# anaykulkarni/collective-communication-mpi

Measured on AMD Instinct MI355X. Metric: all-reduce algbw (GB/s) @1GiB fp32 + DP4xTP2 fwd step time, 1/2/4/8 MI355X, higher is better.
Workload: dtype fp32; 1 GPU; global_batch=2048, seq_len=16, parallelism=dp1xtp1, allreduce_algo=twoshot, allreduce_bytes=1073741824

## Files before the change

### collective_communication_mpi_amd/csrc/device/attn_common.hpp

```cpp
#pragma once
#include <cstdint>

#include <hip/hip_runtime.h>

namespace ccmpi {
namespace dev {
namespace attn {

struct AttnArgs {
  const uint16_t* qkv;
  uint16_t* o;
  float* lse;
  const uint16_t* dout;
  uint16_t* dqkv;
  float* dbias;
  int B, S, Hl, D, ld_qkv, ld_o;
  float scale;
  uint16_t* pool;
  int ld_pool;
  int dout_bstride;
  int dout_rstride;
  const uint16_t* wo;
  int ld_wo, n_out;
  float* zp;
  int ld_zp;
  const float* bo;
  const uint16_t* dz;
  int ld_dz;
  float dz_scale;
  float* ztok;
  int ld_zt;
  int zrows;
  float* zpush[16];
  const uint16_t* xq;
  int ld_xq, kq;
  const uint16_t* wq;
  int ld_wq;
  const float* bq;
  uint16_t* qkv_out;
  const float* img;
  uint16_t* xq_out;
  const float* fold_wq;
  int ld_fold_wq;
  const float* fold_we;
  int ld_fold_we;
  uint16_t* fold_out;
  int ld_fold_out, fold_R, fold_d, fold_kp;
  int fold_at_start;
  int fold_sched;
  unsigned long long* tstamp;
};
constexpr int kTStamps = 32;

bool mfma_supported(const AttnArgs& a, bool bwd);
void launch_fwd_mfma(const AttnArgs& a, hipStream_t stream);
void launch_bwd_mfma(const AttnArgs& a, hipStream_t stream);
void launch_qkv_fwd_mfma(const AttnArgs& a, hipStream_t stream);
extern int g_qkv_grid_cap;
extern int g_qkv_fold_sched;
extern int g_qkv_fold_grid;
extern int g_bwd_grid_cap;

}
}
}
```

### collective_communication_mpi_amd/csrc/device/attn_mfma.hip

```cpp
#include <hip/hip_runtime.h>

#include <algorithm>
#include <cstdlib>

#include "attn_common.hpp"
#include "common.hpp"

namespace ccmpi {
namespace dev {
void fold_emb_qkv_mfma(const float* Wq, int ld_wq, const float* We, int ld_we, uint16_t* Weff, int ld_eff, int R, int d,
                       int kp, hipStream_t stream);
namespace attn {
namespace {

typedef __bf16 bf16x8 __attribute__((ext_vector_type(8)));
typedef short s4 __attribute__((ext_vector_type(4)));
typedef float f4 __attribute__((ext_vector_type(4)));
constexpr int WPB = 4;

__device__ __forceinline__ s4 pack4(float a, float b, float c, float d) {
  const uint2 u{pk_bf16(a, b), pk_bf16(c, d)};
  return __builtin_bit_cast(s4, u);
}
__device__ __forceinline__ bf16x8 ld_row16(const uint16_t* p, bool ok) {
// ... 799 lines not shown
    }
    store_tile<D, LD>(Ot, acc, a.scale, gq, a.ld_qkv, S, lane);
  }
  if (a.dbias) {
    float* red = reinterpret_cast<float*>(sm);
    __syncthreads();
#pragma unroll
    for (int nt = 0; nt < NT; ++nt) {
      float q = bq[nt], k = bk[nt], v = bv[nt];
      q = pair32_sum(pair16_sum(q));
      k = pair32_sum(pair16_sum(k));
      v = pair32_sum(pair16_sum(v));
      if (g == 0) {
        red[(wave * 3 + 0) * D + 16 * nt + c] = q;
        red[(wave * 3 + 1) * D + 16 * nt + c] = k;
        red[(wave * 3 + 2) * D + 16 * nt + c] = v;
      }
    }
    __syncthreads();
    for (int i = threadIdx.x; i < 3 * D; i += blockDim.x) {
      float acc = 0.f;
#pragma unroll
      for (int w = 0; w < WPB; ++w) acc += red[w * 3 * D + i];
      atomicAdd(a.dbias + (i / D) * HD + h * D + i % D, acc);
    }
  }
}

template <int D>
constexpr size_t bwd_lds_bytes() {
  return (size_t)WPB * 4 * 16 * (D + 8) * sizeof(uint16_t);
}

int grid_for(int npairs, int cap, int nw = WPB) { return std::max(1, std::min((npairs + nw - 1) / nw, cap)); }

}

bool mfma_supported(const AttnArgs& a, bool bwd) {
  if (a.S < 1 || a.S > 16 || !(a.D == 32 || a.D == 64 || a.D == 128)) return false;
  if (a.ld_qkv % 8 || a.ld_o % 8 || ((uint64_t)a.qkv % 16) || ((uint64_t)a.o % 16)) return false;
  if (bwd && (a.dout_bstride % 8 || a.dout_rstride % 8 || ((uint64_t)a.dout % 16) || ((uint64_t)a.dqkv % 16))) return false;
  return true;
}

void launch_fwd_mfma(const AttnArgs& a, hipStream_t stream) {
  const int grid = grid_for(a.B * a.Hl, 4096);
  if (a.D == 32) hipLaunchKernelGGL(k_attn16_fwd<32>, dim3(grid), dim3(256), 0, stream, a);
  else if (a.D == 64) hipLaunchKernelGGL(k_attn16_fwd<64>, dim3(grid), dim3(256), 0, stream, a);
  else hipLaunchKernelGGL(k_attn16_fwd<128>, dim3(grid), dim3(256), 0, stream, a);
}

int g_qkv_grid_cap = std::getenv("CCMPI_QKV_GRID") ? std::atoi(std::getenv("CCMPI_QKV_GRID")) : 256;

constexpr double kFoldRounds = 1.5;
int g_qkv_fold_sched = -1;
int g_qkv_fold_grid = 1;

bool fold_sched_on() {
  if (g_qkv_fold_sched < 0) {
    const char* e = std::getenv("CCMPI_QKV_FOLD_SCHED");
    g_qkv_fold_sched = (e && std::atoi(e) == 0) ? 0 : 1;
  }
  return g_qkv_fold_sched != 0;
}

int fold_sched_for(const AttnArgs& a, int grid) {
// ... 36 lines not shown
  const dim3 block(64 * kQkvWaves);
  AttnArgs a = args;
  const bool fold_apart = a.fold_out && fold_tiles_n > grid;
  if (fold_apart) a.fold_out = nullptr;
  a.fold_sched = fold_sched_for(a, grid);
  const bool train = a.lse || a.qkv_out || a.xq_out || a.pool;
  const bool lean = a.ld_wq == 72 && (!a.fold_out || a.fold_at_start);
  if (a.tstamp) launch_qkv_variant<true, true, false>(a, grid, block, stream);
  else if (lean) (train ? launch_qkv_variant<false, true, true> : launch_qkv_variant<false, false, true>)(a, grid, block, stream);
  else (train ? launch_qkv_variant<false, true, false> : launch_qkv_variant<false, false, false>)(a, grid, block, stream);
  if (fold_apart)
    fold_emb_qkv_mfma(args.fold_wq, args.ld_fold_wq, args.fold_we, args.ld_fold_we, args.fold_out, args.ld_fold_out,
                      args.fold_R, args.fold_d, args.fold_kp, stream);
}

int g_bwd_grid_cap = 0;

void launch_bwd_mfma(const AttnArgs& a, hipStream_t stream) {
  int grid = grid_for(a.B * a.Hl, a.dbias ? (g_bwd_grid_cap > 0 ? g_bwd_grid_cap : 256 * a.Hl) : 4096);
  grid = std::max(a.Hl, grid / a.Hl * a.Hl);
  if (a.D == 32) {
    hipLaunchKernelGGL(k_attn16_bwd<32>, dim3(grid), dim3(256), bwd_lds_bytes<32>(), stream, a);
  } else if (a.D == 64) {
    hipLaunchKernelGGL(k_attn16_bwd<64>, dim3(grid), dim3(256), bwd_lds_bytes<64>(), stream, a);
  } else {
    static bool attr = hipFuncSetAttribute(reinterpret_cast<const void*>(k_attn16_bwd<128>),
                                           hipFuncAttributeMaxDynamicSharedMemorySize,
                                           (int)bwd_lds_bytes<128>()) == hipSuccess;
    (void)attr;
    hipLaunchKernelGGL(k_attn16_bwd<128>, dim3(grid), dim3(256), bwd_lds_bytes<128>(), stream, a);
  }
}

}
}
}
```

### collective_communication_mpi_amd/csrc/device/attn_small.hip

```cpp
#include <pybind11/pybind11.h>
#include <pybind11/stl.h>

#include <tuple>
#include <vector>

#include "attn_common.hpp"
#include "common.hpp"
#include "ops.hpp"

namespace ccmpi {
namespace dev {

namespace {
using attn::AttnArgs;

__device__ __forceinline__ float ld_bf16(const uint16_t* p) { return __uint_as_float((uint32_t)(*p) << 16); }
__device__ __forceinline__ void st_bf16(uint16_t* p, float v) { *p = (uint16_t)f32_to_bf16_bits(v); }

__device__ __forceinline__ float wave_max(float v) {
  for (int o = 32; o > 0; o >>= 1) v = fmaxf(v, __shfl_xor(v, o));
  return v;
}
__device__ __forceinline__ float wave_sum(float v) {
  for (int o = 32; o > 0; o >>= 1) v += __shfl_xor(v, o);
// ... 162 lines not shown
        atomicAdd(&colsum[2 * D + d], dv);
      }
    }
  }
  if (a.dbias && fixed_col && threadIdx.x < S * D) {
    const int d = threadIdx.x % D;
    atomicAdd(&colsum[d], sq);
    atomicAdd(&colsum[D + d], sk);
    atomicAdd(&colsum[2 * D + d], sv);
  }
  if (a.dbias) {
    __syncthreads();
    for (int c = threadIdx.x; c < 3 * D; c += blockDim.x) {
      const int part = c / D, d = c % D;
      atomicAdd(a.dbias + part * HD + h * D + d, colsum[c]);
    }
  }
}

size_t fwd_lds(int S, int D) { return sizeof(float) * (3 * S * (D + 1) + S * (S + 1)); }
size_t bwd_lds(int S, int D) { return sizeof(float) * (5 * S * (D + 1) + 2 * S * (S + 1) + S + 3 * D); }

void check_dims(int S, int D, bool bwd) {
  if (S < 1 || S > 64 || D < 1 || D > 256) throw std::invalid_argument("attn_small: need 1 <= S <= 64, D <= 256");
  if ((bwd ? bwd_lds(S, D) : fwd_lds(S, D)) > 160 * 1024) throw std::invalid_argument("attn_small: tile exceeds LDS");
}

static void check_fused_fc(const AttnArgs& a, bool bwd) {
  if (!attn::mfma_supported(a, bwd) || a.n_out < 1 || a.n_out > 16 || 4 % a.Hl || !a.wo)
    throw std::invalid_argument("attention: fused fc_o needs S <= 16, D in {32, 64, 128}, Hl | 4, n_out <= 16");
  if (bwd && (a.ld_dz < 16 || a.ld_dz % 8 || ((uint64_t)a.dz % 16)))
    throw std::invalid_argument("attention: fused fc_o backward needs dz rows of >= 16 bf16, 16-B aligned");
  if (!bwd && !a.pool) throw std::invalid_argument("attention: fused fc_o forward needs the pooled output");
}

void attn_fwd(uint64_t qkv, uint64_t o, uint64_t lse, int B, int S, int Hl, int D, int ld_qkv, int ld_o, float scale,
              uint64_t pool, int ld_pool, uint64_t stream, uint64_t wo, int ld_wo, int n_out, uint64_t zp, int ld_zp,
              uint64_t bo, uint64_t ztok, int ld_zt, int zrows, const std::vector<uint64_t>& zpush) {
  check_dims(S, D, false);
  AttnArgs a{(const uint16_t*)qkv, (uint16_t*)o, (float*)lse, nullptr, nullptr, nullptr, B, S, Hl, D, ld_qkv, ld_o, scale,
             (uint16_t*)pool, ld_pool, 0, 0, (const uint16_t*)wo, ld_wo, n_out, (float*)zp, ld_zp, (const float*)bo,
             nullptr, 0, 1.0f};
  if (zp) check_fused_fc(a, false);
  if (ztok || zrows) {
    if (zp || !attn::mfma_supported(a, false) || n_out < 1 || n_out > 16 || 4 % Hl || !wo || ld_wo % 8 ||
        (wo % 16) || ld_zt < 16 || ld_zt % 4 || (ztok % 16))
      throw std::invalid_argument("attention: per-token fused fc_o needs S <= 16, D in {32, 64, 128}, Hl | 4, "
                                  "n_out <= 16, 16-B aligned W_o rows, z rows of >= 16 floats");
    if (zrows) {
      const int64_t M = (int64_t)B * S;
      const int64_t blocks = M / zrows;
      if (zrows % S || M % zrows || blocks < 1 || blocks > 16 || (int64_t)zpush.size() != blocks)
        throw std::invalid_argument("attention: push fc_o needs whole sequences per block (zrows % S == 0), "
                                    "B*S = blocks x zrows and one target per block (<= 16)");
      for (int64_t j = 0; j < blocks; ++j) {
        if (!zpush[j] || zpush[j] % 16) throw std::invalid_argument("attention: push fc_o targets must be 16-B aligned");
        a.zpush[j] = reinterpret_cast<float*>(zpush[j]);
      }
    }
    a.ztok = reinterpret_cast<float*>(ztok);
    a.ld_zt = ld_zt;
    a.zrows = zrows;
  }
  if (attn::mfma_supported(a, false)) {
    attn::launch_fwd_mfma(a, (hipStream_t)stream);
    CCMPI_HIP_CHECK(hipGetLastError());
// ... 30 lines not shown
  a.lse = (float*)lse;
  a.tstamp = (unsigned long long*)tstamp;
  a.B = B; a.S = S; a.Hl = Hl; a.D = D; a.ld_qkv = ld_qkv; a.scale = scale;
  a.pool = (uint16_t*)pool; a.ld_pool = ld_pool;
  a.wo = (const uint16_t*)wo; a.ld_wo = ld_wo; a.n_out = n_out; a.bo = (const float*)bo;
  a.xq = (const uint16_t*)xq; a.ld_xq = ld_xq; a.kq = kq;
  a.wq = (const uint16_t*)wq; a.ld_wq = ld_wq; a.bq = (const float*)bq; a.qkv_out = (uint16_t*)qkv_out;
  a.img = (const float*)img; a.xq_out = (uint16_t*)xq_out;
  a.zp = (float*)zmean; a.ld_zp = ld_zmean;
  a.fold_wq = (const float*)fold_wq; a.ld_fold_wq = ld_fold_wq; a.fold_we = (const float*)fold_we;
  a.ld_fold_we = ld_fold_we; a.fold_out = (uint16_t*)fold_out; a.ld_fold_out = ld_fold_out;
  a.fold_R = fold_R; a.fold_d = fold_d; a.fold_kp = kq;
  static const int at_start = std::getenv("CCMPI_FOLD_TAIL_AT") && std::string(std::getenv("CCMPI_FOLD_TAIL_AT")) == "end" ? 0 : 1;
  a.fold_at_start = at_start;
  a.ztok = (float*)ztok; a.ld_zt = ld_zt; a.zrows = zrows;
  if (zrows) {
    const int64_t M = (int64_t)B * S;
    const int64_t blocks = M / zrows;
    if (zrows % S || M % zrows || blocks < 1 || blocks > 16 || (int64_t)zpush.size() != blocks)
      throw std::invalid_argument("attention: push fc_o needs whole sequences per block (zrows % S == 0), "
                                  "B*S = blocks x zrows and one target per block (<= 16)");
    for (int64_t j = 0; j < blocks; ++j) {
      if (!zpush[j] || zpush[j] % 16) throw std::invalid_argument("attention: push fc_o targets must be 16-B aligned");
      a.zpush[j] = reinterpret_cast<float*>(zpush[j]);
    }
  }
  if (B == 0) return;
  attn::launch_qkv_fwd_mfma(a, (hipStream_t)stream);
  CCMPI_HIP_CHECK(hipGetLastError());
}

void attn_bwd(uint64_t qkv, uint64_t o, uint64_t lse, uint64_t dout, uint64_t dqkv, uint64_t dbias, int B, int S,
              int Hl, int D, int ld_qkv, int ld_o, float scale, int dout_bstride, int dout_rstride, uint64_t stream,
              uint64_t dz, int ld_dz, uint64_t wo, int ld_wo, int n_out, float dz_scale) {
  check_dims(S, D, true);
  AttnArgs a{(const uint16_t*)qkv, (uint16_t*)o, (float*)lse, (const uint16_t*)dout, (uint16_t*)dqkv, (float*)dbias,
             B, S, Hl, D, ld_qkv, ld_o, scale, nullptr, 0, dout_bstride, dout_rstride, (const uint16_t*)wo, ld_wo,
             n_out, nullptr, 0, nullptr, (const uint16_t*)dz, ld_dz, dz_scale};
  if (dz) check_fused_fc(a, true);
  if (attn::mfma_supported(a, true)) {
    attn::launch_bwd_mfma(a, (hipStream_t)stream);
    CCMPI_HIP_CHECK(hipGetLastError());
    return;
  }
  hipLaunchKernelGGL(k_attn_bwd, dim3(B * Hl), dim3(256), bwd_lds(S, D), (hipStream_t)stream, a);
  CCMPI_HIP_CHECK(hipGetLastError());
}

constexpr int kMaxT = 4, kTT = 32;
struct TRegions {
  uint64_t off[kMaxT], rows[kMaxT], cols[kMaxT];
  uint16_t* dst[kMaxT];
  int tiles[kMaxT + 1];
  int n;
};

__device__ __forceinline__ bool in_regions(const TRegions& tr, uint64_t i) {
  for (int k = 0; k < tr.n; ++k)
    if (i >= tr.off[k] && i - tr.off[k] < tr.rows[k] * tr.cols[k]) return true;
  return false;
}

struct AdamArgs {
  float* p;
  float* g;
  float* m;
  float* v;
  uint16_t* p16;
  uint64_t n;
  float lr, b1, b2, eps, wd, bc1, bc2, grad_scale;
  int zero_grad;
  int* step_dev;
// ... 207 lines not shown
void register_attn_ops(pybind11::module_& m) {
  m.def("rows_mean", &rows_mean, "out[g] = mean of fp32 rows z[g S .. g S + S) (ordered sum)", pybind11::arg("z"),
        pybind11::arg("ld_z"), pybind11::arg("out"), pybind11::arg("ld_out"), pybind11::arg("groups"),
        pybind11::arg("S"), pybind11::arg("ncol"), pybind11::arg("stream"),
        pybind11::call_guard<pybind11::gil_scoped_release>());
  m.def("attn_set_qkv_grid", [](int cap) { attn::g_qkv_grid_cap = cap > 0 ? cap : 256; },
        "workgroups of the fused QKV forward (default 256: one 8-wave workgroup per CU)", pybind11::arg("cap"));
  m.def("attn_set_qkv_fold_sched", [](int v) { attn::g_qkv_fold_sched = v < 0 ? -1 : (v ? 1 : 0); },
        "fused QKV forward with the in-kernel fold: 1 = fold owners take fewer pair blocks, 0 = grid-stride, "
        "-1 = CCMPI_QKV_FOLD_SCHED (default 1)", pybind11::arg("v"));
  m.def("attn_set_qkv_fold_grid", [](int v) { attn::g_qkv_fold_grid = v ? 1 : 0; },
        "fused QKV forward with the in-kernel fold: 1 = at small batches the grid grows by the fold's tiles "
        "(fold-only workgroups beside the attention ones), 0 = not (ranks sharing one GPU)", pybind11::arg("v"));
  m.def("attn_set_bwd_grid", [](int cap) { attn::g_bwd_grid_cap = cap > 0 ? cap : 0; },
        "backward kernel grid cap (tuning)");
  namespace py = pybind11;
  m.def("attn_small_fwd", &attn_fwd, py::arg("qkv"), py::arg("o"), py::arg("lse"), py::arg("B"), py::arg("S"),
        py::arg("Hl"), py::arg("D"), py::arg("ld_qkv"), py::arg("ld_o"), py::arg("scale"), py::arg("pool"),
        py::arg("ld_pool"), py::arg("stream"), py::arg("wo") = 0, py::arg("ld_wo") = 0, py::arg("n_out") = 0,
        py::arg("zp") = 0, py::arg("ld_zp") = 0, py::arg("bo") = 0, py::arg("ztok") = 0, py::arg("ld_zt") = 16,
        py::arg("zrows") = 0, py::arg("zpush") = std::vector<uint64_t>{}, py::call_guard<py::gil_scoped_release>());
  m.def("attn_qkv_fwd", &attn_qkv_fwd, py::arg("xq"), py::arg("ld_xq"), py::arg("kq"), py::arg("wq"), py::arg("ld_wq"),
        py::arg("bq"), py::arg("qkv_out"), py::arg("ld_qkv"), py::arg("lse"), py::arg("B"), py::arg("S"), py::arg("Hl"),
        py::arg("D"), py::arg("scale"), py::arg("pool"), py::arg("ld_pool"), py::arg("wo"), py::arg("ld_wo"),
        py::arg("n_out"), py::arg("bo"), py::arg("ztok"), py::arg("ld_zt"), py::arg("zrows"), py::arg("zpush"),
        py::arg("stream"), py::arg("img") = 0, py::arg("xq_out") = 0, py::arg("zmean") = 0, py::arg("ld_zmean") = 16,
        py::arg("fold_wq") = 0, py::arg("ld_fold_wq") = 0, py::arg("fold_we") = 0, py::arg("ld_fold_we") = 0,
        py::arg("fold_out") = 0, py::arg("ld_fold_out") = 0, py::arg("fold_R") = 0, py::arg("fold_d") = 0,
        py::arg("tstamp") = 0, py::call_guard<py::gil_scoped_release>());
  m.def("attn_small_bwd", &attn_bwd, py::arg("qkv"), py::arg("o"), py::arg("lse"), py::arg("dout"), py::arg("dqkv"),
        py::arg("dbias"), py::arg("B"), py::arg("S"), py::arg("Hl"), py::arg("D"), py::arg("ld_qkv"), py::arg("ld_o"),
        py::arg("scale"), py::arg("dout_bstride"), py::arg("dout_rstride"), py::arg("stream"), py::arg("dz") = 0,
        py::arg("ld_dz") = 0, py::arg("wo") = 0, py::arg("ld_wo") = 0, py::arg("n_out") = 0,
        py::arg("dz_scale") = 1.0f, py::call_guard<py::gil_scoped_release>());
  m.def("adamw_step", &adamw, py::arg("p"), py::arg("g"), py::arg("m"), py::arg("v"), py::arg("p16"), py::arg("n"),
        py::arg("lr"), py::arg("b1"), py::arg("b2"), py::arg("eps"), py::arg("wd"), py::arg("step"),
        py::arg("grad_scale"), py::arg("stream"),
        py::arg("tregions") = std::vector<std::tuple<uint64_t, uint64_t, uint64_t, uint64_t>>{},
        py::arg("zero_grad") = false, py::arg("step_dev") = 0, py::arg("step_parity") = 0, py::call_guard<py::gil_scoped_release>());
  m.def("cast_bf16", &cast_bf16, py::arg("x"), py::arg("y"), py::arg("n"), py::arg("stream"),
        py::arg("tregions") = std::vector<std::tuple<uint64_t, uint64_t, uint64_t, uint64_t>>{},
        py::call_guard<py::gil_scoped_release>());
  m.def("patchify", &patchify, py::arg("x"), py::arg("xp"), py::arg("B"), py::arg("img"), py::arg("p"), py::arg("kp"),
        py::arg("stream"), py::arg("ldo") = 0, py::call_guard<py::gil_scoped_release>());
}

}
}
```

### collective_communication_mpi_amd/models/mnist_tp.py

```python
from __future__ import annotations

import math
import os
from dataclasses import dataclass
from typing import Optional

import numpy as np
import torch

from .. import _native
from ..ops import gemm_nt, gemm_tn, transpose
from ..parallel.dp import FlatParams, GradBuckets
from ..parallel.layout import device_group_for, get_info, naive_collect_backward_output, naive_collect_backward_x, \
    naive_collect_forward_input, naive_collect_forward_output


@dataclass
class LayerConfig:
    d_model: int = 768
    d_attn: int = 256
    n_heads: int = 4
    n_classes: int = 10
    img: int = 28
    patch: int = 7
# ... 160 lines not shown

class MnistTPLayer:
    def __init__(self, comm, cfg: LayerConfig, device=None):
        self.cfg = cfg
        self.comm = comm
        world, rank = comm.Get_size(), comm.Get_rank()
        if cfg.tp * cfg.dp != world:
            raise ValueError(f"tp*dp = {cfg.tp * cfg.dp} != world size {world}")
        if cfg.n_heads % cfg.tp:
            raise ValueError("n_heads must be divisible by tp")
        self.tp_idx, self.dp_idx, self.mp_comm, self.dp_comm, _, _ = get_info(
            comm, rank, cfg.tp, cfg.dp, "fc_q", cfg.d_model, cfg.d_attn)
        self.device = torch.device(device) if device is not None else torch.device("cuda", torch.cuda.current_device())
        self.tp_dev = device_group_for(self.mp_comm) if cfg.tp > 1 else None
        self.dp_dev = device_group_for(self.dp_comm) if cfg.dp > 1 else None
        self.hl = cfg.n_heads // cfg.tp
        self.hd = self.hl * cfg.head_dim
        d = cfg.d_model
        specs = [
            ("o_w", (cfg.out_pad, self.hd)), ("o_b", (cfg.out_pad,)),
            ("qkv_w", (3 * self.hd, d)), ("qkv_b", (3 * self.hd,)),
            ("emb_w", (d, cfg.kp)),
        ]
        grad_alloc = (lambda n: self.dp_dev.zeros(n, torch.float32)) if self.dp_dev is not None else None
        transposed = [n for n, used in (("qkv_w", cfg.emb_grad == "dh" and cfg.plain_gemm == "own"),
                                         ("o_w", not self._fused_fc_o_bwd())) if used]
        self.flat = FlatParams(specs, self.device, grad_alloc, transposed=transposed)
        self.buckets = GradBuckets(self.flat, self.dp_dev, [["o_w", "o_b"], ["qkv_w", "qkv_b"],
                                                            ["emb_w"]],
                                   algo=cfg.dp_algo, overlap=cfg.overlap)
        self._load(full_init(cfg))
        self._bufs = {}
        self._hx = None
        self._fold_next = None
        self._hx_ld = (cfg.d_model + cfg.kp + 63) // 64 * 64

    def _load(self, w):
        cfg, t = self.cfg, self.tp_idx
        sl = slice(t * self.hd, (t + 1) * self.hd)
        P = self.flat.param
        P("emb_w").copy_(w["emb_w"])
        P("qkv_w").copy_(torch.cat([w["q_w"][sl], w["k_w"][sl], w["v_w"][sl]]))
        P("qkv_b").copy_(torch.cat([w["q_b"][sl], w["k_b"][sl], w["v_b"][sl]]))
        ow = torch.zeros(cfg.out_pad, self.hd)
        ow[: cfg.n_classes] = w["o_w"][:, sl]
        P("o_w").copy_(ow)
        ob = torch.zeros(cfg.out_pad)
        ob[: cfg.n_classes] = w["o_b"]
        P("o_b").copy_(ob)
        self.flat.refresh_bf16()

    def gathered_full(self):
        cfg = self.cfg
        hc = self.mp_comm.comm if hasattr(self.mp_comm, "comm") else self.mp_comm
        parts = hc.allgather({k: self.flat.param(k).detach().cpu() for k in ("qkv_w", "qkv_b", "o_w")})
        q = torch.cat([p["qkv_w"][: self.hd] for p in parts])
        return {"q_w": q, "o_w": torch.cat([p["o_w"][: cfg.n_classes] for p in parts], dim=1),
                "emb_w": self.flat.param("emb_w").detach().cpu()}

    def _buf(self, name, shape, dtype, symmetric_on=None):
        key = (name, tuple(shape), dtype)
        b = self._bufs.get(key)
        if b is None:
            b = symmetric_on.empty(shape, dtype) if symmetric_on is not None else torch.empty(
                shape, dtype=dtype, device=self.device)
            self._bufs[key] = b
# ... 421 lines not shown
        G = self.flat.grad
        P16 = self.flat.param16
        D = _native.device()
        st = torch.cuda.current_stream(self.device).cuda_stream
        fused = dlogits is None
        if not fused:
            G("o_b")[: cfg.n_classes].add_(dlogits.sum(0))
        if (cfg.fc_o_mode == "naive" and cfg.tp > 1) or (cfg.fc_o_mode == "token" and not self._fused_fc_o_bwd()):
            dz = self._buf("dz", (M, cfg.out_pad), torch.bfloat16)
            dz.zero_()
            dz.view(B, S, cfg.out_pad)[:, :, : cfg.n_classes] = (dlogits / S).unsqueeze(1).to(torch.bfloat16)
            datt = self._buf("datt", (M, self.hd), torch.bfloat16)
            if cfg.fc_o_mode == "token":
                gemm_tn(dz, att, out=G("o_w"), accumulate=True)
                gemm_nt(dz, self.flat.param16_t("o_w"), out=datt)
            else:
                self._backward_naive_fc_o(dz, datt, B)
            dout, dout_b, dout_r = datt, S * datt.stride(0), datt.stride(0)
        else:
            dzp = self._buf("dzp", (B, cfg.out_pad), torch.bfloat16)
            if not fused:
                dzp.zero_()
                dzp[:, : cfg.n_classes] = dlogits.to(torch.bfloat16)
            if not (fused and getattr(self, "_dwo_done", False)):
                gemm_tn(dzp, pool, out=G("o_w"), accumulate=True, splitk=max(1, min(32, B // 64)))
            self._dwo_done = False
            if self._fused_fc_o_bwd():
                dout, dout_b, dout_r = None, 0, 0
            else:
                dpool = self._buf("dpool", (B, self.hd), torch.bfloat16)
                gemm_nt(dzp, self.flat.param16_t("o_w"), out=dpool, alpha=1.0 / S)
                dout, dout_b, dout_r = dpool, dpool.stride(0), 0
        self.buckets.ready(0)
        dqkv = self._buf("dqkv", (M, 3 * self.hd), torch.bfloat16)
        fc = {}
        if dout is None:
            dzp = self._buf("dzp", (B, cfg.out_pad), torch.bfloat16)
            wo = P16("o_w")
            fc = dict(dz=dzp.data_ptr(), ld_dz=dzp.stride(0), wo=wo.data_ptr(), ld_wo=wo.stride(0), n_out=cfg.out_pad,
                      dz_scale=1.0 / S)
        D.attn_small_bwd(qkv.data_ptr(), 0 if att is None else att.data_ptr(), lse.data_ptr(),
                         0 if dout is None else dout.data_ptr(),
                         dqkv.data_ptr(), G("qkv_b").data_ptr(), B, S, self.hl, cfg.head_dim, qkv.stride(0),
                         self.hd if att is None else att.stride(0),
                         1.0 / math.sqrt(cfg.head_dim), dout_b, dout_r, st, **fc)
        if cfg.emb_grad == "reassoc" and cfg.qkv_grad == "reassoc":
            key = ("a_emb2", 3 * self.hd, cfg.kp)
            if key not in self._bufs:
                self._bufs[key] = torch.zeros(2, 3 * self.hd, cfg.kp, dtype=torch.float32, device=self.device)
                self._a_idx = 0
            a, a_next = self._bufs[key][self._a_idx], self._bufs[key][self._a_idx ^ 1]
            self._a_idx ^= 1
            gemm_tn(dqkv, xp, out=a, accumulate=True, workspace=False)
            tp = self.tp_dev is not None
            ge = self._buf("gemb", (d, cfg.kp), torch.float32, self.tp_dev) if tp else G("emb_w")
            we, wq, gq = self.flat.param("emb_w"), self.flat.param("qkv_w"), G("qkv_w")
            if tp:
                ge.zero_()
            D.emb_qkv_wgrad(a.data_ptr(), a.stride(0), we.data_ptr(), we.stride(0), wq.data_ptr(), wq.stride(0),
                            gq.data_ptr(), gq.stride(0), ge.data_ptr(), ge.stride(0), a_next.data_ptr(),
                            a_next.stride(0), 3 * self.hd, d, cfg.kp, st)
            self.buckets.ready(1)
            if tp:
                self.tp_dev.allreduce(ge, ge, "SUM")
                G("emb_w").add_(ge)
            self.buckets.ready(2)
            return
        if cfg.emb_grad == "reassoc" and self._hx is not None:
            a = self._buf("a_emb", (3 * self.hd, cfg.kp), torch.float32)
            gemm_tn(dqkv, self._hx, out=G("qkv_w"), accumulate=True, tail=a)
            self.buckets.ready(1)
            self._emb_grad_reassoc(dqkv, xp, a=a)
            self.buckets.ready(2)
            return
        gemm_tn(dqkv, h, out=G("qkv_w"), accumulate=True)
        self.buckets.ready(1)
        if cfg.emb_grad == "reassoc":
            self._emb_grad_reassoc(dqkv, xp)
            self.buckets.ready(2)
            return
        dh = self._buf("dh", (M, d), torch.bfloat16)
        if cfg.plain_gemm == "hipblaslt":
            torch.matmul(dqkv, P16("qkv_w"), out=dh)
        else:
            gemm_nt(dqkv, self.flat.param16_t("qkv_w"), out=dh)
        if self.tp_dev is not None:
            gpart = self._buf("gemb", (d, cfg.kp), torch.float32, self.tp_dev)
            gemm_tn(dh, xp, out=gpart)
            self.tp_dev.allreduce(gpart, gpart, "SUM")
            G("emb_w").add_(gpart)
        else:
            gemm_tn(dh, xp, out=G("emb_w"), accumulate=True)
        self.buckets.ready(2)

    def _emb_grad_reassoc(self, dqkv, xp, a=None) -> None:
        cfg = self.cfg
        d = cfg.d_model
        if a is None:
            a = self._buf("a_emb", (3 * self.hd, cfg.kp), torch.float32)
            gemm_tn(dqkv, xp, out=a)
        w = self.flat.param("qkv_w")
        G = self.flat.grad
        if self.tp_dev is not None:
            gpart = self._buf("gemb", (d, cfg.kp), torch.float32, self.tp_dev)
            torch.mm(w.t(), a, out=gpart)
            self.tp_dev.allreduce(gpart, gpart, "SUM")
            G("emb_w").add_(gpart)
        else:
            G("emb_w").addmm_(w.t(), a)

    def _backward_naive_fc_o(self, dz, datt, B):
        cfg = self.cfg
        S = cfg.seq
        att_full, w_sh = self._naive
        k = cfg.out_pad // cfg.tp
        dz_local = naive_collect_backward_output(dz.view(B, S, cfg.out_pad), self.tp_idx, cfg.tp)
        dz_local = dz_local.reshape(B * S, k).contiguous()
        gw_sh = gemm_tn(dz_local, att_full)
        gw_full = torch.zeros(cfg.out_pad, cfg.d_attn, dtype=torch.float32, device=self.device)
        gw_full[self.tp_idx * k:(self.tp_idx + 1) * k] = gw_sh
        self.tp_dev.allreduce(gw_full, gw_full, "SUM")
        self.flat.grad("o_w").add_(gw_full[:, self.tp_idx * self.hd:(self.tp_idx + 1) * self.hd])
        dx_full = gemm_nt(dz_local, transpose(w_sh), out_dtype=torch.bfloat16)
        dx = naive_collect_backward_x(dx_full.view(B, S, cfg.d_attn), self.mp_comm, cfg.tp)
        datt.copy_(dx.reshape(B * S, self.hd))

    def zero_grad(self) -> None:
# ... 21 lines not shown
```

Before: 3229 GB/s.

## Fuse A = dQKV^T Xp weight-grad GEMM into attention backward kernel

Adds a new attention backward kernel that, alongside dQ/dK/dV, accumulates the reassociated weight-gradient product dQKV^T·Xp in registers. It writes per-workgroup partial slabs to a workspace, and a separate reduce kernel sums them into A in a fixed order. The goal is to avoid materialising dQKV in HBM and running a separate gemm_tn over it. In exchange it uses more LDS, block-wide syncs per step, an extra reduction pass and a workspace. The path is enabled by default when shapes qualify. The measured metric is all-reduce bandwidth plus forward step time, so this backward-only change may not show up in it.

```diff
diff --git a/collective_communication_mpi_amd/csrc/device/attn_common.hpp b/collective_communication_mpi_amd/csrc/device/attn_common.hpp
--- a/collective_communication_mpi_amd/csrc/device/attn_common.hpp
+++ b/collective_communication_mpi_amd/csrc/device/attn_common.hpp
@@ -49,16 +49,25 @@
   int fold_at_start;
   int fold_sched;
   unsigned long long* tstamp;
+  const uint16_t* xp;
+  int ld_xp, kp;
+  float* a_out;
+  int ld_a;
+  float* a_ws;
 };
 constexpr int kTStamps = 32;
 
 bool mfma_supported(const AttnArgs& a, bool bwd);
 void launch_fwd_mfma(const AttnArgs& a, hipStream_t stream);
 void launch_bwd_mfma(const AttnArgs& a, hipStream_t stream);
+bool bwd_wgrad_supported(const AttnArgs& a);
+size_t bwd_wgrad_ws_bytes(int B, int Hl, int D, int ld_a);
+void launch_bwd_wgrad_mfma(const AttnArgs& a, hipStream_t stream);
 void launch_qkv_fwd_mfma(const AttnArgs& a, hipStream_t stream);
 extern int g_qkv_grid_cap;
 extern int g_qkv_fold_sched;
 extern int g_qkv_fold_grid;
+extern int g_bwd_wg_grid_cap;
 extern int g_bwd_grid_cap;
 
 }
diff --git a/collective_communication_mpi_amd/csrc/device/attn_mfma.hip b/collective_communication_mpi_amd/csrc/device/attn_mfma.hip
--- a/collective_communication_mpi_amd/csrc/device/attn_mfma.hip
+++ b/collective_communication_mpi_amd/csrc/device/attn_mfma.hip
@@ -855,6 +855,317 @@
   return (size_t)WPB * 4 * 16 * (D + 8) * sizeof(uint16_t);
 }
 
+
+__device__ __forceinline__ bf16x8 tr8(const uint16_t* p, int ld) {
+  typedef __attribute__((address_space(3))) s4* lds_s4;
+  const s4 x0 = __builtin_amdgcn_ds_read_tr16_b64_v4i16((lds_s4)(p));
+  const s4 x1 = __builtin_amdgcn_ds_read_tr16_b64_v4i16((lds_s4)(p + 4 * ld));
+  typedef short s8 __attribute__((ext_vector_type(8)));
+  return __builtin_bit_cast(bf16x8, (s8)__builtin_shufflevector(x0, x1, 0, 1, 2, 3, 4, 5, 6, 7));
+}
+
+template <int LD>
+__device__ __forceinline__ s4 tile_b_tr(const uint16_t* T, int lane, int col0) {
+  typedef __attribute__((address_space(3))) s4* lds_s4;
+  const int g = lane >> 4, tq = (lane >> 2) & 3, tp = lane & 3;
+  return __builtin_amdgcn_ds_read_tr16_b64_v4i16((lds_s4)(T + (4 * g + tq) * LD + col0 + 4 * tp));
+}
+
+template <int D>
+__device__ __forceinline__ void keep_tile_t(uint16_t* T, const f4 (&v)[D / 16], float mul, int lane) {
+  const int c = lane & 15, g = lane >> 4;
+  __builtin_amdgcn_wave_barrier();
+#pragma unroll
+  for (int nt = 0; nt < D / 16; ++nt)
+    *reinterpret_cast<uint2*>(T + (16 * nt + c) * 16 + 4 * g) =
+        uint2{pk_bf16(v[nt][0] * mul, v[nt][1] * mul), pk_bf16(v[nt][2] * mul, v[nt][3] * mul)};
+}
+
+template <int CTRL, int BANKS = 0xf>
+__device__ __forceinline__ float dpp_mov(float old, float v) {
+  return __int_as_float(__builtin_amdgcn_update_dpp(__float_as_int(old), __float_as_int(v), CTRL, 0xf, BANKS, false));
+}
+__device__ __forceinline__ float row16_sum_prod(float p, float q) {
+  const float x = __fmul_rn(p, q);
+  float s = __fmaf_rn(p, q, dpp_mov<0xB1>(0.f, x));
+  s = s + dpp_mov<0x4E>(0.f, s);
+  s = s + dpp_mov<0x12C, 0x5>(dpp_mov<0x124, 0xA>(0.f, s), s);
+  return s + dpp_mov<0x128>(0.f, s);
+}
+
+template <int D, int NXT, int NW>
+__global__ void __launch_bounds__(64 * NW) k_attn16_bwd_wg(AttnArgs a) {
+  constexpr int LD = D + 8, NK = D / 32, NT = D / 16, TILE = 16 * LD, LDX = 16 * NXT;
+  constexpr int WST = 4 * TILE + 16 * LDX;
+  constexpr int TG = NT, KG = NW / TG, SPG = NW / KG, KS = SPG / 2;
+  static_assert(NW % TG == 0 && SPG % 2 == 0, "k-groups of whole k-steps (two sequences each)");
+  static_assert((WST * 2) % 16 == 0 && (TILE * 2) % 16 == 0, "16-B aligned tiles");
+  static_assert(NW * 3 * D * 4 <= NW * WST * 2 && TG * 3 * NXT * 1024 <= NW * WST * 2,
+                "the end's reductions fit the tiles");
+  extern __shared__ __attribute__((aligned(16))) uint16_t sm[];
+  const int wave = threadIdx.x >> 6, lane = threadIdx.x & 63, c = lane & 15, g = lane >> 4;
+  uint16_t* T0 = sm + wave * WST;
+  uint16_t* T1 = T0 + TILE;
+  uint16_t* T2 = T1 + TILE;
+  uint16_t* Ot = T2 + TILE;
+  uint16_t* X = Ot + TILE;
+  uint16_t* wos = sm + NW * WST;
+  const int HD = a.Hl * D;
+  float bq[NT], bk[NT], bv[NT];
+#pragma unroll
+  for (int nt = 0; nt < NT; ++nt) bq[nt] = bk[nt] = bv[nt] = 0.f;
+  const int h = blockIdx.x % a.Hl, nbh = gridDim.x / a.Hl;
+  if (a.dz) {
+    for (int i = threadIdx.x; i < 16 * D; i += blockDim.x) {
+      const int cls = i / D;
+      wos[i] = cls < a.n_out ? a.wo[(size_t)cls * a.ld_wo + h * D + i % D] : (uint16_t)0;
+    }
+    __syncthreads();
+  }
+  uint32_t wcol[8];
+#pragma unroll
+  for (int q = 0; q < 8; ++q)
+    wcol[q] = (a.dz && lane < D) ? (uint32_t)wos[2 * q * D + lane] | ((uint32_t)wos[(2 * q + 1) * D + lane] << 16) : 0u;
+  const int tg = wave % TG, kg = wave / TG, tq = (lane >> 2) & 3, tp = lane & 3;
+  const int nxt = (a.kp + 15) >> 4, nch = a.kp >> 3;
+  f4 wacc[3][NXT];
+#pragma unroll
+  for (int j = 0; j < 3; ++j)
+#pragma unroll
+    for (int xt = 0; xt < NXT; ++xt) wacc[j][xt] = f4{0.f, 0.f, 0.f, 0.f};
+  struct In {
+    bf16x8 q[NK], k[NK], v[NK], d[NK];
+    uint32_t z;
+    float lc, lr[4];
+  };
+  auto load = [&](In& in, int b0) {
+    const bool live = b0 + wave < a.B;
+    const int b = live ? b0 + wave : a.B - 1;
+    const int S = live ? a.S : 0;
+    const uint16_t* qb = a.qkv + (size_t)b * a.S * a.ld_qkv + h * D;
+#pragma unroll
+    for (int kk = 0; kk < NK; ++kk) {
+      const size_t off = (size_t)c * a.ld_qkv + 32 * kk + 8 * g;
+      in.q[kk] = ld_row16(qb + off, c < S);
+      in.k[kk] = ld_row16(qb + HD + off, c < S);
+      in.v[kk] = ld_row16(qb + 2 * HD + off, c < S);
+    }
+    if (a.dz) {
+      in.z = reinterpret_cast<const uint32_t*>(a.dz + (size_t)b * a.ld_dz)[lane & 7];
+    } else {
+      const uint16_t* db = a.dout + (size_t)b * a.dout_bstride + h * D;
+#pragma unroll
+      for (int kk = 0; kk < NK; ++kk) in.d[kk] = ld_row16(db + (size_t)c * a.dout_rstride + 32 * kk + 8 * g, c < S);
+    }
+    const float* lse = a.lse + ((size_t)b * a.Hl + h) * a.S;
+    in.lc = c < S ? lse[c] : 0.f;
+#pragma unroll
+    for (int r = 0; r < 4; ++r) in.lr[r] = (4 * g + r < S) ? lse[4 * g + r] : 0.f;
+  };
+  const int bfirst = (blockIdx.x / a.Hl) * NW, bstep = nbh * NW;
+  In nx;
+  if (bfirst < a.B) load(nx, bfirst);
+  for (int b0 = bfirst; b0 < a.B; b0 += bstep) {
+    const bool live = b0 + wave < a.B;
+    const int b = live ? b0 + wave : a.B - 1;
+    const int S = live ? a.S : 0;
+    In in = nx;
+    if (b0 + bstep < a.B) load(nx, b0 + bstep);
+    bf16x8(&qr)[NK] = in.q, (&kr)[NK] = in.k, (&vr)[NK] = in.v, (&dr)[NK] = in.d;
+    uint4 xv[3];
+#pragma unroll
+    for (int t = 0; t < 3; ++t) {
+      const int p = lane + 64 * t, row = p / nch, ch = p - row * nch;
+      xv[t] = row < S ? *reinterpret_cast<const uint4*>(a.xp + ((size_t)b * a.S + row) * a.ld_xp + 8 * ch) : uint4{0, 0, 0, 0};
+    }
+    if (a.dz) {
+      float v = 0.f;
+#pragma unroll
+      for (int q = 0; q < 8; ++q) {
+        const uint32_t zw = __builtin_amdgcn_readlane(in.z, q);
+        v += bf16_lo(zw) * bf16_lo(wcol[q]);
+        v += bf16_hi(zw) * bf16_hi(wcol[q]);
+      }
+      if (lane < D) T2[lane] = (uint16_t)f32_to_bf16_bits(v * a.dz_scale);
+      __builtin_amdgcn_wave_barrier();
+#pragma unroll
+      for (int kk = 0; kk < NK; ++kk) dr[kk] = ld_row16(T2 + 32 * kk + 8 * g, c < S);
+      __builtin_amdgcn_wave_barrier();
+    }
+    put_rows<D, LD>(T1, qr, lane);
+    put_rows<D, LD>(T0, kr, lane);
+    put_rows<D, LD>(T2, dr, lane);
+    const float lse_c = in.lc;
+    const float(&lse_r)[4] = in.lr;
+    f4 sT = {0.f, 0.f, 0.f, 0.f}, sM = sT, dpT = sT, dpM = sT;
+#pragma unroll
+    for (int kk = 0; kk < NK; ++kk) {
+      sT = mma32(kr[kk], qr[kk], sT);
+      sM = mma32(qr[kk], kr[kk], sM);
+      dpT = mma32(vr[kk], dr[kk], dpT);
+      dpM = mma32(dr[kk], vr[kk], dpM);
+    }
+    float P[4], PT[4], dS[4], dST[4];
+    float dl = 0.f, dl_r[4];
+#pragma unroll
+    for (int r = 0; r < 4; ++r) {
+      const bool ok = (4 * g + r < S) && (c < S);
+      PT[r] = ok ? __expf(sT[r] * a.scale - lse_c) : 0.f;
+      P[r] = ok ? __expf(sM[r] * a.scale - lse_r[r]) : 0.f;
+      dl += PT[r] * dpT[r];
+      dl_r[r] = row16_sum_prod(P[r], dpM[r]);
+    }
+    dl = pair32_sum(pair16_sum(dl));
+#pragma unroll
+    for (int r = 0; r < 4; ++r) {
+      dST[r] = PT[r] * (dpT[r] - dl);
+      dS[r] = P[r] * (dpM[r] - dl_r[r]);
+    }
+    __builtin_amdgcn_wave_barrier();
+    const s4 aP = pack4(P[0], P[1], P[2], P[3]);
+    const s4 aDS = pack4(dS[0], dS[1], dS[2], dS[3]);
+    const s4 aDST = pack4(dST[0], dST[1], dST[2], dST[3]);
+    f4 acc[NT];
+    uint16_t* gq = a.dqkv ? a.dqkv + (size_t)b * a.S * a.ld_qkv + h * D : nullptr;
+#pragma unroll
+    for (int nt = 0; nt < NT; ++nt) {
+      acc[nt] = mma16(aP, tile_b_tr<LD>(T2, lane, 16 * nt), f4{0.f, 0.f, 0.f, 0.f});
+      bv[nt] += acc[nt][0] + acc[nt][1] + acc[nt][2] + acc[nt][3];
+    }
+    if (gq) store_tile<D, LD>(Ot, acc, 1.f, gq + 2 * HD, a.ld_qkv, S, lane);
+    keep_tile_t<D>(T2, acc, 1.f, lane);
+#pragma unroll
+    for (int nt = 0; nt < NT; ++nt) {
+      acc[nt] = mma16(aDS, tile_b_tr<LD>(T1, lane, 16 * nt), f4{0.f, 0.f, 0.f, 0.f});
+      bk[nt] += a.scale * (acc[nt][0] + acc[nt][1] + acc[nt][2] + acc[nt][3]);
+    }
+    if (gq) store_tile<D, LD>(Ot, acc, a.scale, gq + HD, a.ld_qkv, S, lane);
+    keep_tile_t<D>(T1, acc, a.scale, lane);
+#pragma unroll
+    for (int nt = 0; nt < NT; ++nt) {
+      acc[nt] = mma16(aDST, tile_b_tr<LD>(T0, lane, 16 * nt), f4{0.f, 0.f, 0.f, 0.f});
+      bq[nt] += a.scale * (acc[nt][0] + acc[nt][1] + acc[nt][2] + acc[nt][3]);
+    }
+    if (gq) store_tile<D, LD>(Ot, acc, a.scale, gq, a.ld_qkv, S, lane);
+    keep_tile_t<D>(T0, acc, a.scale, lane);
+#pragma unroll
+    for (int t = 0; t < 3; ++t) {
+      const int p = lane + 64 * t, row = p / nch, ch = p - row * nch;
+      if (row < 16) *reinterpret_cast<uint4*>(X + row * LDX + 8 * ch) = xv[t];
+    }
+    __syncthreads();
+#pragma unroll
+    for (int u = 0; u < KS; ++u) {
+      const uint16_t* W = sm + (kg * SPG + 2 * u + (g >> 1)) * WST;
+      const int r0 = 8 * (g & 1) + tq;
+      bf16x8 af[3];
+#pragma unroll
+      for (int j = 0; j < 3; ++j)
+        af[j] = *reinterpret_cast<const bf16x8*>(W + j * TILE + (16 * tg + c) * 16 + 8 * (g & 1));
+#pragma unroll
+      for (int xt = 0; xt < NXT; ++xt) {
+        if (xt < nxt) {
+          const bf16x8 bf = tr8(W + 4 * TILE + r0 * LDX + 16 * xt + 4 * tp, LDX);
+#pragma unroll
+          for (int j = 0; j < 3; ++j) wacc[j][xt] = mma32(af[j], bf, wacc[j][xt]);
+        }
+      }
+    }
+    __syncthreads();
+  }
+  if (a.dbias) {
+    float* red = reinterpret_cast<float*>(sm);
+#pragma unroll
+    for (int nt = 0; nt < NT; ++nt) {
+      float q = bq[nt], k = bk[nt], v = bv[nt];
+      q = pair32_sum(pair16_sum(q));
+      k = pair32_sum(pair16_sum(k));
+      v = pair32_sum(pair16_sum(v));
+      if (g == 0) {
+        red[(wave * 3 + 0) * D + 16 * nt + c] = q;
+        red[(wave * 3 + 1) * D + 16 * nt + c] = k;
+        red[(wave * 3 + 2) * D + 16 * nt + c] = v;
+      }
+    }
+    __syncthreads();
+    for (int i = threadIdx.x; i < 3 * D; i += blockDim.x) {
+      float acc = 0.f;
+#pragma unroll
+      for (int w = 0; w < NW; ++w) acc += red[w * 3 * D + i];
+      atomicAdd(a.dbias + (i / D) * HD + h * D + i % D, acc);
+    }
+    __syncthreads();
+  }
+  float* part = reinterpret_cast<float*>(sm) + (size_t)tg * 3 * NXT * 256;
+  for (int k = 1; k < KG; ++k) {
+    if (kg == k) {
+#pragma unroll
+      for (int j = 0; j < 3; ++j)
+#pragma unroll
+        for (int xt = 0; xt < NXT; ++xt)
+#pragma unroll
+          for (int r = 0; r < 4; ++r) part[((j * NXT + xt) * 4 + r) * 64 + lane] = wacc[j][xt][r];
+    }
+    __syncthreads();
+    if (kg == 0) {
+#pragma unroll
+      for (int j = 0; j < 3; ++j)
+#pragma unroll
+        for (int xt = 0; xt < NXT; ++xt)
+#pragma unroll
+          for (int r = 0; r < 4; ++r) wacc[j][xt][r] += part[((j * NXT + xt) * 4 + r) * 64 + lane];
+    }
+    __syncthreads();
+  }
+  if (kg == 0) {
+    float* dst = a.a_ws ? a.a_ws + (size_t)(blockIdx.x / a.Hl) * 3 * HD * a.ld_a : a.a_out;
+#pragma unroll
+    for (int j = 0; j < 3; ++j)
+#pragma unroll
+      for (int xt = 0; xt < NXT; ++xt) {
+        if (16 * xt + c < a.kp) {
+#pragma unroll
+          for (int r = 0; r < 4; ++r) {
+            float* p = dst + (size_t)(j * HD + h * D + 16 * tg + 4 * g + r) * a.ld_a + 16 * xt + c;
+            if (a.a_ws) *p = wacc[j][xt][r];
+            else atomicAdd(p, wacc[j][xt][r]);
+          }
+        }
+      }
+  }
+}
+
+__global__ void __launch_bounds__(256) k_a_reduce(const float* __restrict__ ws, int nslab, float* __restrict__ out, int n,
+                                                  int ld_a, int kp) {
+  __shared__ float4 part[4][64];
+  const int col = threadIdx.x & 63, q = threadIdx.x >> 6, i = (blockIdx.x * 64 + col) * 4;
+  const bool ok = i < n && i % ld_a < kp;
+  float4 acc = {0.f, 0.f, 0.f, 0.f};
+  if (ok) {
+#pragma unroll 4
+    for (int p = q; p < nslab; p += 4) {
+      const float4 v = *reinterpret_cast<const float4*>(ws + (size_t)p * n + i);
+      acc.x += v.x; acc.y += v.y; acc.z += v.z; acc.w += v.w;
+    }
+  }
+  part[q][col] = acc;
+  __syncthreads();
+  if (q == 0 && ok) {
+    float4 o = *reinterpret_cast<float4*>(out + i);
+#pragma unroll
+    for (int k = 1; k < 4; ++k) {
+      acc.x += part[k][col].x; acc.y += part[k][col].y; acc.z += part[k][col].z; acc.w += part[k][col].w;
+    }
+    o.x += acc.x; o.y += acc.y; o.z += acc.z; o.w += acc.w;
+    *reinterpret_cast<float4*>(out + i) = o;
+  }
+}
+
+template <int D, int NXT, int NW>
+constexpr size_t bwd_wg_lds_bytes() {
+  return (size_t)NW * (4 * 16 * (D + 8) + 16 * 16 * NXT) * sizeof(uint16_t) + 16 * D * sizeof(uint16_t);
+}
+
 int grid_for(int npairs, int cap, int nw = WPB) { return std::max(1, std::min((npairs + nw - 1) / nw, cap)); }
 
 }
@@ -957,6 +1268,44 @@
   }
 }
 
-}
-}
-}
+bool bwd_wgrad_supported(const AttnArgs& a) {
+  if (!mfma_supported(a, true) || !(a.D == 32 || a.D == 64)) return false;
+  if (a.kp < 8 || a.kp > 96 || a.kp % 8 || a.ld_xp % 8 || a.ld_xp < a.kp || a.ld_a % 4 || a.ld_a < a.kp) return false;
+  if (!a.xp || !a.a_out || ((uint64_t)a.xp % 16) || ((uint64_t)a.a_out % 16) || ((uint64_t)a.a_ws % 16)) return false;
+  return true;
+}
+
+int g_bwd_wg_grid_cap = 256;
+constexpr int kWgWaves = 8;
+static int bwd_wg_grid(int B, int Hl) {
+  const int grid = grid_for(B * Hl, g_bwd_wg_grid_cap, kWgWaves);
+  return std::max(Hl, grid / Hl * Hl);
+}
+
+size_t bwd_wgrad_ws_bytes(int B, int Hl, int D, int ld_a) {
+  return (size_t)(bwd_wg_grid(B, Hl) / Hl) * 3 * Hl * D * ld_a * sizeof(float);
+}
+
+template <int D, int NXT>
+static void launch_bwd_wg(const AttnArgs& a, int grid, hipStream_t stream) {
+  constexpr size_t lds = bwd_wg_lds_bytes<D, NXT, kWgWaves>();
+  static bool attr = hipFuncSetAttribute(reinterpret_cast<const void*>(k_attn16_bwd_wg<D, NXT, kWgWaves>),
+                                         hipFuncAttributeMaxDynamicSharedMemorySize, (int)lds) == hipSuccess;
+  (void)attr;
+  hipLaunchKernelGGL((k_attn16_bwd_wg<D, NXT, kWgWaves>), dim3(grid), dim3(64 * kWgWaves), lds, stream, a);
+}
+
+void launch_bwd_wgrad_mfma(const AttnArgs& a, hipStream_t stream) {
+  const int grid = bwd_wg_grid(a.B, a.Hl);
+  const bool wide = a.kp > 80;
+  if (a.D == 32) (wide ? launch_bwd_wg<32, 6> : launch_bwd_wg<32, 5>)(a, grid, stream);
+  else (wide ? launch_bwd_wg<64, 6> : launch_bwd_wg<64, 5>)(a, grid, stream);
+  if (a.a_ws) {
+    const int n = 3 * a.Hl * a.D * a.ld_a;
+    hipLaunchKernelGGL(k_a_reduce, dim3((n / 4 + 63) / 64), dim3(256), 0, stream, a.a_ws, grid / a.Hl, a.a_out, n, a.ld_a, a.kp);
+  }
+}
+
+}
+}
+}
diff --git a/collective_communication_mpi_amd/csrc/device/attn_small.hip b/collective_communication_mpi_amd/csrc/device/attn_small.hip
--- a/collective_communication_mpi_amd/csrc/device/attn_small.hip
+++ b/collective_communication_mpi_amd/csrc/device/attn_small.hip
@@ -218,6 +218,19 @@
   if (bwd && (a.ld_dz < 16 || a.ld_dz % 8 || ((uint64_t)a.dz % 16)))
     throw std::invalid_argument("attention: fused fc_o backward needs dz rows of >= 16 bf16, 16-B aligned");
   if (!bwd && !a.pool) throw std::invalid_argument("attention: fused fc_o forward needs the pooled output");
+}
+
+static void check_fused_wgrad(const AttnArgs& a) {
+  if (!attn::bwd_wgrad_supported(a))
+    throw std::invalid_argument("attention: the fused A = dQKV^T Xp needs S <= 16, D in {32, 64}, kp % 8 == 0 in [8, 96], "
+                                "ld_xp % 8 == 0 and >= kp, ld_a % 4 == 0 and >= kp, 16-B aligned xp, a_out and workspace");
+}
+
+bool attn_bwd_wgrad_supported(int S, int D, int kp, int ld_xp, uint64_t xp, uint64_t a_out, int ld_a, int ld_qkv) {
+  AttnArgs a{};
+  a.S = S; a.D = D; a.ld_qkv = ld_qkv; a.kp = kp; a.ld_xp = ld_xp; a.ld_a = ld_a;
+  a.xp = (const uint16_t*)xp; a.a_out = (float*)a_out;
+  return attn::bwd_wgrad_supported(a);
 }
 
 void attn_fwd(uint64_t qkv, uint64_t o, uint64_t lse, int B, int S, int Hl, int D, int ld_qkv, int ld_o, float scale,
@@ -314,12 +327,22 @@
 
 void attn_bwd(uint64_t qkv, uint64_t o, uint64_t lse, uint64_t dout, uint64_t dqkv, uint64_t dbias, int B, int S,
               int Hl, int D, int ld_qkv, int ld_o, float scale, int dout_bstride, int dout_rstride, uint64_t stream,
-              uint64_t dz, int ld_dz, uint64_t wo, int ld_wo, int n_out, float dz_scale) {
+              uint64_t dz, int ld_dz, uint64_t wo, int ld_wo, int n_out, float dz_scale, uint64_t xp, int ld_xp, int kp,
+              uint64_t a_out, int ld_a, uint64_t a_ws) {
   check_dims(S, D, true);
   AttnArgs a{(const uint16_t*)qkv, (uint16_t*)o, (float*)lse, (const uint16_t*)dout, (uint16_t*)dqkv, (float*)dbias,
              B, S, Hl, D, ld_qkv, ld_o, scale, nullptr, 0, dout_bstride, dout_rstride, (const uint16_t*)wo, ld_wo,
              n_out, nullptr, 0, nullptr, (const uint16_t*)dz, ld_dz, dz_scale};
   if (dz) check_fused_fc(a, true);
+  if (a_out) {
+    a.xp = (const uint16_t*)xp; a.ld_xp = ld_xp; a.kp = kp;
+    a.a_out = (float*)a_out; a.ld_a = ld_a; a.a_ws = (float*)a_ws;
+    check_fused_wgrad(a);
+    if (B == 0) return;
+    attn::launch_bwd_wgrad_mfma(a, (hipStream_t)stream);
+    CCMPI_HIP_CHECK(hipGetLastError());
+    return;
+  }
   if (attn::mfma_supported(a, true)) {
     attn::launch_bwd_mfma(a, (hipStream_t)stream);
     CCMPI_HIP_CHECK(hipGetLastError());
@@ -593,7 +616,17 @@
         py::arg("dbias"), py::arg("B"), py::arg("S"), py::arg("Hl"), py::arg("D"), py::arg("ld_qkv"), py::arg("ld_o"),
         py::arg("scale"), py::arg("dout_bstride"), py::arg("dout_rstride"), py::arg("stream"), py::arg("dz") = 0,
         py::arg("ld_dz") = 0, py::arg("wo") = 0, py::arg("ld_wo") = 0, py::arg("n_out") = 0,
-        py::arg("dz_scale") = 1.0f, py::call_guard<py::gil_scoped_release>());
+        py::arg("dz_scale") = 1.0f, py::arg("xp") = 0, py::arg("ld_xp") = 0, py::arg("kp") = 0, py::arg("a_out") = 0,
+        py::arg("ld_a") = 0, py::arg("a_ws") = 0, py::call_guard<py::gil_scoped_release>());
+  m.def("attn_bwd_wgrad_supported", &attn_bwd_wgrad_supported,
+        "whether attn_small_bwd takes a_out (A += dQKV^T Xp in the backward kernel) at this shape", py::arg("S"),
+        py::arg("D"), py::arg("kp"), py::arg("ld_xp"), py::arg("xp"), py::arg("a_out"), py::arg("ld_a"),
+        py::arg("ld_qkv") = 0);
+  m.def("attn_bwd_wgrad_ws_bytes", &attn::bwd_wgrad_ws_bytes,
+        "bytes of the a_ws workspace (per-workgroup partial slabs, summed in a fixed order) for this launch shape",
+        py::arg("B"), py::arg("Hl"), py::arg("D"), py::arg("ld_a"));
+  m.def("attn_set_bwd_wg_grid", [](int cap) { attn::g_bwd_wg_grid_cap = cap > 0 ? cap : 256; },
+        "workgroups of the backward with the fused A (default 256: one 8-wave workgroup per CU)", py::arg("cap"));
   m.def("adamw_step", &adamw, py::arg("p"), py::arg("g"), py::arg("m"), py::arg("v"), py::arg("p16"), py::arg("n"),
         py::arg("lr"), py::arg("b1"), py::arg("b2"), py::arg("eps"), py::arg("wd"), py::arg("step"),
         py::arg("grad_scale"), py::arg("stream"),
diff --git a/collective_communication_mpi_amd/models/mnist_tp.py b/collective_communication_mpi_amd/models/mnist_tp.py
--- a/collective_communication_mpi_amd/models/mnist_tp.py
+++ b/collective_communication_mpi_amd/models/mnist_tp.py
@@ -216,6 +216,7 @@
         self._load(full_init(cfg))
         self._bufs = {}
         self._hx = None
+        self._bwd_fuse_a = os.environ.get("CCMPI_BWD_FUSE_A", "1") != "0"
         self._fold_next = None
         self._hx_ld = (cfg.d_model + cfg.kp + 63) // 64 * 64
 
@@ -703,26 +704,36 @@
                 gemm_nt(dzp, self.flat.param16_t("o_w"), out=dpool, alpha=1.0 / S)
                 dout, dout_b, dout_r = dpool, dpool.stride(0), 0
         self.buckets.ready(0)
-        dqkv = self._buf("dqkv", (M, 3 * self.hd), torch.bfloat16)
-        fc = {}
-        if dout is None:
-            dzp = self._buf("dzp", (B, cfg.out_pad), torch.bfloat16)
-            wo = P16("o_w")
-            fc = dict(dz=dzp.data_ptr(), ld_dz=dzp.stride(0), wo=wo.data_ptr(), ld_wo=wo.stride(0), n_out=cfg.out_pad,
-                      dz_scale=1.0 / S)
-        D.attn_small_bwd(qkv.data_ptr(), 0 if att is None else att.data_ptr(), lse.data_ptr(),
-                         0 if dout is None else dout.data_ptr(),
-                         dqkv.data_ptr(), G("qkv_b").data_ptr(), B, S, self.hl, cfg.head_dim, qkv.stride(0),
-                         self.hd if att is None else att.stride(0),
-                         1.0 / math.sqrt(cfg.head_dim), dout_b, dout_r, st, **fc)
-        if cfg.emb_grad == "reassoc" and cfg.qkv_grad == "reassoc":
+        reassoc = cfg.emb_grad == "reassoc" and cfg.qkv_grad == "reassoc"
+        a = a_next = None
+        if reassoc:
             key = ("a_emb2", 3 * self.hd, cfg.kp)
             if key not in self._bufs:
                 self._bufs[key] = torch.zeros(2, 3 * self.hd, cfg.kp, dtype=torch.float32, device=self.device)
                 self._a_idx = 0
             a, a_next = self._bufs[key][self._a_idx], self._bufs[key][self._a_idx ^ 1]
             self._a_idx ^= 1
-            gemm_tn(dqkv, xp, out=a, accumulate=True, workspace=False)
+        ws = self._bwd_fuse_a_ws(B, xp, a, qkv) if reassoc else None
+        fuse_a = ws is not None
+        dqkv = None if fuse_a else self._buf("dqkv", (M, 3 * self.hd), torch.bfloat16)
+        fc = {}
+        if fuse_a:
+            fc = dict(xp=xp.data_ptr(), ld_xp=xp.stride(0), kp=cfg.kp, a_out=a.data_ptr(), ld_a=a.stride(0),
+                      a_ws=ws.data_ptr())
+        if dout is None:
+            dzp = self._buf("dzp", (B, cfg.out_pad), torch.bfloat16)
+            wo = P16("o_w")
+            fc.update(dz=dzp.data_ptr(), ld_dz=dzp.stride(0), wo=wo.data_ptr(), ld_wo=wo.stride(0), n_out=cfg.out_pad,
+                      dz_scale=1.0 / S)
+        D.attn_small_bwd(qkv.data_ptr(), 0 if att is None else att.data_ptr(), lse.data_ptr(),
+                         0 if dout is None else dout.data_ptr(),
+                         0 if dqkv is None else dqkv.data_ptr(), G("qkv_b").data_ptr(), B, S, self.hl, cfg.head_dim,
+                         qkv.stride(0),
+                         self.hd if att is None else att.stride(0),
+                         1.0 / math.sqrt(cfg.head_dim), dout_b, dout_r, st, **fc)
+        if reassoc:
+            if not fuse_a:
+                gemm_tn(dqkv, xp, out=a, accumulate=True, workspace=False)
             tp = self.tp_dev is not None
             ge = self._buf("gemb", (d, cfg.kp), torch.float32, self.tp_dev) if tp else G("emb_w")
             we, wq, gq = self.flat.param("emb_w"), self.flat.param("qkv_w"), G("qkv_w")
@@ -764,6 +775,19 @@
             gemm_tn(dh, xp, out=G("emb_w"), accumulate=True)
         self.buckets.ready(2)
 
+    def _bwd_fuse_a_ws(self, B, xp, a, qkv):
+        if not self._bwd_fuse_a:
+            return None
+        cfg = self.cfg
+        key = ("a_ws", B, xp.stride(0), xp.data_ptr() % 16, a.data_ptr() % 16, qkv.stride(0))
+        if key not in self._bufs:
+            D = _native.device()
+            ok = D.attn_bwd_wgrad_supported(cfg.seq, cfg.head_dim, cfg.kp, xp.stride(0), xp.data_ptr(), a.data_ptr(),
+                                            a.stride(0), qkv.stride(0))
+            n = D.attn_bwd_wgrad_ws_bytes(B, self.hl, cfg.head_dim, a.stride(0)) // 4 if ok else 0
+            self._bufs[key] = torch.empty(n, dtype=torch.float32, device=self.device) if ok else None
+        return self._bufs[key]
+
     def _emb_grad_reassoc(self, dqkv, xp, a=None) -> None:
         cfg = self.cfg
         d = cfg.d_model
```

After: 3225 GB/s (median of 2 runs). About the same (-0.1%).
